# KaffinPX/neptune-core

Hardware: AMD Instinct MI355X
Metric: STARK proofs verified/sec (whole node) + Tip5 perms/sec vs VALU roofline (higher is better)
Workload: dtype u64 (Goldilocks mod p; XFE = cubic extension)

## Files before the change

### include/neptune_hip.h

```cpp
#ifndef NEPTUNE_HIP_H
#define NEPTUNE_HIP_H

#include <stddef.h>
#include <stdint.h>

#ifdef __cplusplus
extern "C" {
#endif

typedef struct nhip_ctx nhip_ctx;

enum {
    NHIP_OK = 0,
    NHIP_ERR_NO_DEVICE = 1,
    NHIP_ERR_HIP = 2,
    NHIP_ERR_OOM = 3,
    NHIP_ERR_ARG = 4,
    NHIP_ERR_DECODE = 5
};

#define NHIP_HW_QUEUES_RECOMMENDED 8
int nhip_init(uint32_t device_mask, nhip_ctx **out);
void nhip_destroy(nhip_ctx *ctx);
const char *nhip_strerror(int code);
// ... 53 lines not shown
} nhip_proof;

typedef struct {
    uint64_t num_proofs, proof_words;
    uint64_t tip5_perms_static;
    uint64_t tip5_perms_merkle;
    double ms_decode, ms_upload;
    double ms_fiat_shamir, ms_row_hash, ms_merkle, ms_ood_air, ms_fri, ms_deep, ms_device_total;
    double ms_merkle_hash;
    uint64_t merkle_hash_launches;
    double ms_mp_hash_kernel;
    uint64_t mp_hash_kernel_launches, mp_hash_kernel_perms;
    double ms_device_decode;
    double ms_mp_hash_exec;
    double ms_row_hash_exec;
} nhip_stats;

typedef struct nhip_air nhip_air;
typedef struct nhip_batch nhip_batch;

void nhip_stark_params_default(nhip_stark_params *out);
int nhip_air_create(const uint64_t *words, size_t n_words, nhip_air **out);
typedef struct {
    uint32_t lds_slots;
    uint32_t step_width;
    uint32_t slot_budget;
} nhip_air_options;
int nhip_air_create_ex(const uint64_t *words, size_t n_words, const nhip_air_options *options, nhip_air **out);
void nhip_air_destroy(nhip_air *air);
int nhip_air_info(const nhip_air *air, uint32_t *num_nodes, uint32_t *num_levels, uint32_t *num_constraints);
int nhip_air_slots(const nhip_air *air, uint32_t *lds_slots, uint32_t *global_slots);
int nhip_air_program(const nhip_air *air, uint32_t *step_off, size_t step_cap, uint32_t *ins, size_t ins_cap,
                     size_t *n_steps, size_t *n_ins);
int nhip_proof_decodes(const nhip_air *air, const nhip_stark_params *params, const nhip_claim *claim,
                       const nhip_proof *proof);
int nhip_host_alloc(size_t bytes, void **out);
int nhip_host_free(void *p);
int nhip_host_register(void *p, size_t bytes);
int nhip_host_unregister(void *p);
int nhip_host_alloc_near(nhip_ctx *ctx, size_t bytes, void **out);
int nhip_device_numa(nhip_ctx *ctx, int *numa_node, int *cpus, size_t cpu_cap, size_t *n_cpus);
int nhip_numa_from_sysfs(const char *sysfs_root, const char *pci_bus_id, int *numa_node, int *cpus, size_t cpu_cap,
                         size_t *n_cpus);
int nhip_cpulist_parse(const char *list, int *cpus, size_t cpu_cap, size_t *n_cpus);
int nhip_host_page_node(const void *ptr);
int nhip_set_host_threads(nhip_ctx *ctx, unsigned threads);
int nhip_verify_batch(nhip_ctx *ctx, nhip_air *air, const nhip_stark_params *params, const nhip_claim *claims,
                      const nhip_proof *proofs, size_t n, uint8_t *verdicts, nhip_stats *stats);
int nhip_batch_prepare(nhip_ctx *ctx, nhip_air *air, const nhip_stark_params *params, const nhip_claim *claims,
                       const nhip_proof *proofs, size_t n, nhip_batch **out);
int nhip_batch_refill(nhip_ctx *ctx, nhip_batch *batch, nhip_air *air, const nhip_stark_params *params,
                      const nhip_claim *claims, const nhip_proof *proofs, size_t n);
int nhip_batch_run(nhip_ctx *ctx, nhip_batch *batch, uint8_t *verdicts, uint8_t *all_ok);
int nhip_batch_launch(nhip_ctx *ctx, nhip_batch *batch);
int nhip_batch_wait(nhip_ctx *ctx, nhip_batch *batch, uint8_t *verdicts, uint8_t *all_ok);
int nhip_batch_stats(const nhip_batch *batch, nhip_stats *stats);
int nhip_batch_set_launch_timing(nhip_batch *batch, int on);
int nhip_batch_set_streams(nhip_batch *batch, int streams);
int nhip_batch_set_graph(nhip_batch *batch, int on);
int nhip_set_fs_form(int form);
int nhip_set_climb_from_ops(int64_t ops);
int nhip_batch_transcript(nhip_ctx *ctx, const nhip_batch *batch, size_t proof, uint64_t *xfe_out, size_t xfe_cap,
                          uint32_t *idx_out, size_t idx_cap, uint32_t *fail_bits, size_t *n_xfe);
void nhip_batch_destroy(nhip_batch *batch);

typedef struct nhip_queue nhip_queue;
// ... 221 lines not shown
```

### neptune-core_amd/csrc/stark_host.cpp

```cpp
#include <hip/hip_runtime.h>

#include <algorithm>
#include <atomic>
#include <chrono>
#include <cstdlib>
#include <cstring>
#include <memory>
#include <mutex>
#include <new>
#include <system_error>
#include <thread>
#include <vector>

#include "../../include/neptune_hip.h"
#include "device_scope.hpp"
#include "host_copy.hpp"
#include "host_numa.hpp"
#include "../../include/nhip_challenge_id.h"
#include "goldilocks.hpp"
#include "kernels.hpp"
#include "stark.hpp"
#include "wire.hpp"

using namespace nhip;
// ... 37 lines not shown
    static const bool on = [] {
        const char* v = nhip::ab_env("NHIP_STAGE_NT");
        return !v || std::strtol(v, nullptr, 10) != 0;
    }();
    return on;
}
unsigned host_threads(uint64_t bytes) {
    unsigned t = nhip::host_threads_env() ? nhip::host_threads_env() : std::thread::hardware_concurrency();
    t = std::max(1u, std::min(t, 16u));
    return bytes < (8ull << 20) ? 1u : t;
}

struct PinnedRanges {
    std::mutex mu;
    std::vector<std::pair<uintptr_t, size_t>> r;
    bool contains(const void* p, size_t bytes) {
        const uintptr_t a = (uintptr_t)p;
        std::lock_guard<std::mutex> g(mu);
        for (const auto& x : r)
            if (a >= x.first && a + bytes <= x.first + x.second && a + bytes >= a) return true;
        return false;
    }
};
PinnedRanges& pinned() {
    static PinnedRanges p;
    return p;
}

}

struct OodProgram {
    std::vector<OodIns> prog;
    std::vector<uint32_t> prog_off;
    std::vector<Xfe> consts;
    uint32_t slots = 0;
    uint32_t width = 0;
};

struct nhip_air {
    StarkDims dims_air{};
    std::vector<AirNode> nodes;
    std::vector<uint32_t> level_off;
    uint4 cons_off{};
    OodProgram progs[2];
    uint32_t lds_cap = AIR_LDS_SLOTS_MAX;
    struct Dev {
        int device;
        OodIns* d_prog[2];
        uint32_t* d_prog_off[2];
        Xfe* d_consts[2];
    };
    std::mutex mu;
    std::vector<Dev> devs;
};

struct VerifyScratch {
    std::mutex mu;
    void* dmem = nullptr;
    size_t dmem_bytes = 0;
    void* dwords = nullptr;
    size_t dwords_bytes = 0;
    void* draw = nullptr;
    size_t draw_bytes = 0;
    hipStream_t main = nullptr, aux = nullptr;
    hipEvent_t ev[STARK_EVENTS] = {};
    bool streams = false;
// ... 76 lines not shown
    d.num_checks = sp->num_collinearity_checks;
    d.num_deep = 3;
    d.log2_expansion = sp->log2_fri_expansion;
    d.num_trace_randomizers = sp->num_collinearity_checks + 2 * 3;
    d.num_sampled = air->dims_air.num_sampled;
    d.num_constraints = air->dims_air.num_constraints;
    D.expansion = 1u << sp->log2_fri_expansion;
    D.mont_words = sp->input_form == NHIP_INPUT_MONTGOMERY ? 1u : 0u;
    if (deep_rows8_lds_bytes(d) > 160 * 1024 - 8192) return false;
    if ((1ull << (log2_u64(d.num_checks) + 1 + d.log2_expansion)) > 4096) return false;
    return true;
}

int air_upload(nhip_ctx* ctx, nhip_air* a, nhip_air::Dev* out) {
    std::lock_guard<std::mutex> g(a->mu);
    const int device = nhip_internal_device(ctx);
    for (const auto& d : a->devs)
        if (d.device == device) {
            *out = d;
            return NHIP_OK;
        }
    nhip_air::Dev d{device, {nullptr, nullptr}, {nullptr, nullptr}, {nullptr, nullptr}};
    auto free_dev = [&]() {
        for (int k = 0; k < 2; ++k) {
            if (d.d_prog[k]) (void)hipFree(d.d_prog[k]);
            if (d.d_prog_off[k]) (void)hipFree(d.d_prog_off[k]);
            if (d.d_consts[k]) (void)hipFree(d.d_consts[k]);
        }
    };
    hipError_t e = hipSuccess;
    for (int k = 0; k < 2 && e == hipSuccess; ++k) {
        const OodProgram& pg = a->progs[k];
        e = hipMalloc(&d.d_prog[k], pg.prog.size() * sizeof(OodIns) + 16);
        if (e == hipSuccess) e = hipMalloc(&d.d_prog_off[k], pg.prog_off.size() * 4 + 4);
        if (e == hipSuccess) e = hipMalloc(&d.d_consts[k], pg.consts.size() * sizeof(Xfe) + 24);
        if (e == hipSuccess && !pg.prog.empty())
            e = hipMemcpy(d.d_prog[k], pg.prog.data(), pg.prog.size() * sizeof(OodIns), hipMemcpyHostToDevice);
        if (e == hipSuccess)
            e = hipMemcpy(d.d_prog_off[k], pg.prog_off.data(), pg.prog_off.size() * 4, hipMemcpyHostToDevice);
        if (e == hipSuccess && !pg.consts.empty())
            e = hipMemcpy(d.d_consts[k], pg.consts.data(), pg.consts.size() * sizeof(Xfe), hipMemcpyHostToDevice);
    }
    if (e != hipSuccess) {
        free_dev();
        return hipfail(e);
    }
    try {
        a->devs.reserve(a->devs.size() + 1);
    } catch (const std::bad_alloc&) {
        free_dev();
        return NHIP_ERR_OOM;
    }
    a->devs.push_back(d);
    *out = d;
    return NHIP_OK;
}

static constexpr uint32_t OOD_STEP_WIDTH = 512;

int ood_program_for(uint32_t n) {
    static const uint32_t lim = [] {
        const char* e = nhip::ab_env("NHIP_OOD_WIDE_PROG_MAX");
        return e ? (uint32_t)std::strtoul(e, nullptr, 10) : 1024u;
    }();
    return n <= lim ? 1 : 0;
}

void air_compile(const nhip_air* a, const std::vector<uint32_t>& cons, uint32_t width, uint32_t slot_budget,
                 OodProgram& pg) {
    pg = OodProgram{};
    pg.width = width;
    const size_t NN = a->nodes.size();
    const auto is_op = [&](size_t i) {
        const uint32_t op = a->nodes[i].op;
        return op == AIR_ADD || op == AIR_SUB || op == AIR_MUL;
    };
    std::vector<uint32_t> corder(NN, UINT32_MAX);
    {
        std::vector<uint32_t> st;
        for (size_t c = 0; c < cons.size(); ++c) {
            st.push_back(cons[c]);
            while (!st.empty()) {
                const uint32_t i = st.back();
                st.pop_back();
                if (corder[i] != UINT32_MAX) continue;
                corder[i] = (uint32_t)c;
                if (is_op(i)) {
                    st.push_back(a->nodes[i].a);
                    st.push_back(a->nodes[i].b);
                }
            }
// ... 35 lines not shown
    std::vector<uint32_t> free_slots, to_free;
    uint32_t next_slot = 0, live = 0;
    std::vector<OodIns> cur, acc_next;
    std::vector<std::pair<int32_t, uint64_t>> key(NN);
    auto retires = [&](uint32_t i) {
        if (!is_op(i)) return 0;
        const uint32_t x = a->nodes[i].a, y = a->nodes[i].b;
        int r = 0;
        if (slotted[x] && remaining[x] == (x == y ? 2u : 1u)) ++r;
        if (slotted[y] && y != x && remaining[y] == 1u) ++r;
        return r;
    };
    auto use = [&](uint32_t o) {
        if (slotted[o] && --remaining[o] == 0) to_free.push_back(ref[o]);
    };
    pg.prog_off.assign(1, 0);
    while (!ready.empty() || !acc_next.empty()) {
        cur.swap(acc_next);
        acc_next.clear();
        for (const OodIns& ins : cur)
            if (slotted[cons[ins.b]]) use(cons[ins.b]);
        for (uint32_t i : ready) key[i] = {-retires(i), ((uint64_t)corder[i] << 32) | i};
        std::sort(ready.begin(), ready.end(), [&](uint32_t x, uint32_t y) { return key[x] < key[y]; });
        const size_t room = width > cur.size() ? width - cur.size() : 1;
        std::vector<uint32_t> chosen, rest;
        for (uint32_t i : ready) {
            if (chosen.size() < room && (live < budget || key[i].first < 0 || chosen.empty())) {
                chosen.push_back(i);
                ++live;
            } else {
                rest.push_back(i);
            }
        }
        ready.swap(rest);
        for (uint32_t i : chosen) {
            uint32_t sl;
            if (!free_slots.empty()) {
                sl = free_slots.back();
                free_slots.pop_back();
            } else {
                sl = next_slot++;
            }
            const AirNode& nd = a->nodes[i];
            if (nd.op == AIR_INPUT) {
                cur.push_back(OodIns{OOD_LOAD, OOD_REF_INPUT | (nd.a << 27) | nd.b, 0, sl});
            } else if (nd.op == AIR_CONST) {
                cur.push_back(OodIns{OOD_LOAD, OOD_REF_CONST | cidx[i], 0, sl});
            } else {
                cur.push_back(OodIns{nd.op, ref[nd.a], ref[nd.b], sl});
                use(nd.a);
                use(nd.b);
            }
            ref[i] = OOD_REF_SLOT | sl;
            for (uint32_t c : acc_of[i]) acc_next.push_back(OodIns{OOD_ACC, ref[i], c, 0});
        }
        for (uint32_t i : chosen)
            for (uint32_t k = uoff[i]; k < uoff[i + 1]; ++k)
                if (--deps[users[k]] == 0) ready.push_back(users[k]);
        live -= (uint32_t)to_free.size();
        free_slots.insert(free_slots.end(), to_free.begin(), to_free.end());
        to_free.clear();
        auto kind_rank = [](uint32_t op) {
            return op == OOD_LOAD || op == OOD_ACC ? 0 : (op == AIR_MUL ? 1 : (op == AIR_ADD ? 2 : 3));
        };
        std::stable_sort(cur.begin(), cur.end(),
                         [&](const OodIns& x, const OodIns& y) { return kind_rank(x.op) < kind_rank(y.op); });
        pg.prog.insert(pg.prog.end(), cur.begin(), cur.end());
        pg.prog_off.push_back((uint32_t)pg.prog.size());
        cur.clear();
    }
    for (OodIns& ins : pg.prog)
        if (ins.op == OOD_ACC) ins.dst = next_slot + ins.b;
    pg.slots = next_slot + (uint32_t)cons.size();
}

inline size_t al(size_t x) { return (x + 255) & ~(size_t)255; }

inline size_t grown(size_t need, size_t have, bool refilled) {
    if (!refilled) return need;
    return std::max(need + need / 4, have ? 2 * have : 0);
}

}

extern "C" {

void nhip_stark_params_default(nhip_stark_params* out) {
    if (!out) return;
    out->security_level = 160;
    out->log2_fri_expansion = 2;
    out->num_collinearity_checks = 80;
    out->num_main = 379;
    out->num_aux = 88;
    out->num_quotient_segments = 4;
    out->input_form = NHIP_INPUT_CANONICAL;
}

int nhip_air_create(const uint64_t* w, size_t n, nhip_air** out) { return nhip_air_create_ex(w, n, nullptr, out); }

int nhip_air_create_ex(const uint64_t* w, size_t n, const nhip_air_options* opt, nhip_air** out) {
    if (!w || !out || n < 9) return NHIP_ERR_ARG;
    *out = nullptr;
    const nhip_air_options o = opt ? *opt : nhip_air_options{0, 0, 0};
// ... 84 lines not shown
    if (num_nodes) *num_nodes = (uint32_t)a->nodes.size();
    if (num_levels) *num_levels = (uint32_t)a->level_off.size() - 1;
    if (num_constraints) *num_constraints = a->dims_air.num_constraints;
    return NHIP_OK;
}

int nhip_air_slots(const nhip_air* a, uint32_t* lds_slots, uint32_t* global_slots) {
    if (!a) return NHIP_ERR_ARG;
    const uint32_t l = std::min<uint32_t>(a->progs[0].slots, a->lds_cap);
    if (lds_slots) *lds_slots = l;
    if (global_slots) *global_slots = a->progs[0].slots - l;
    return NHIP_OK;
}

int nhip_air_program(const nhip_air* a, uint32_t* step_off, size_t step_cap, uint32_t* ins, size_t ins_cap,
                     size_t* n_steps, size_t* n_ins) {
    if (!a) return NHIP_ERR_ARG;
    const OodProgram& pg = a->progs[0];
    const size_t ns = pg.prog_off.size() - 1, ni = pg.prog.size();
    if (n_steps) *n_steps = ns;
    if (n_ins) *n_ins = ni;
    if (step_off) {
        if (step_cap < ns + 1) return NHIP_ERR_ARG;
        std::memcpy(step_off, pg.prog_off.data(), (ns + 1) * 4);
    }
    if (ins) {
        if (ins_cap < 4 * ni) return NHIP_ERR_ARG;
        for (size_t i = 0; i < ni; ++i) {
            ins[4 * i] = pg.prog[i].op;
            ins[4 * i + 1] = pg.prog[i].a;
            ins[4 * i + 2] = pg.prog[i].b;
            ins[4 * i + 3] = pg.prog[i].dst;
        }
    }
    return NHIP_OK;
}

int nhip_proof_decodes(const nhip_air* air, const nhip_stark_params* sp, const nhip_claim* claim,
                       const nhip_proof* proof) {
    Dims D{};
    if (!claim || !proof || (proof->len && !proof->words) || !dims_from(sp, air, D)) return -NHIP_ERR_ARG;
    ProofDesc pd;
    FsOp ops[fs_ops_for(MAX_FRI_ROUNDS)];
    uint64_t perms, perms_lcw;
    const ClaimLoc cl{0, (uint32_t)claim->input_len, (uint32_t)claim->output_len};
    const uint32_t f = D.mont_words ? decode_stream<true>(proof->words, 0, proof->len, cl, D, pd, ops, perms, perms_lcw)
                                    : decode_stream<false>(proof->words, 0, proof->len, cl, D, pd, ops, perms, perms_lcw);
    return f ? 0 : 1;
}

namespace {
int batch_prepare(nhip_ctx* ctx, nhip_air* air, const nhip_stark_params* sp, const nhip_claim* claims,
                  const nhip_proof* proofs, const WireSrc* wire, size_t n, nhip_batch** out, VerifyScratch* scr,
                  nhip_batch* reuse = nullptr) {
    if (wire) {
        if (proofs || !sp || sp->input_form != NHIP_INPUT_CANONICAL) return NHIP_ERR_ARG;
        if ((wire->n_bytes && !wire->bytes) || (n && !wire->spans)) return NHIP_ERR_ARG;
        if (!wire_spans_ok(wire->spans, n, wire->n_bytes)) return NHIP_ERR_ARG;
    }
    if (!ctx || !out || (n && (!claims || (!proofs && !wire)))) return NHIP_ERR_ARG;
    if (reuse && (reuse->in_flight || reuse->scratch)) return NHIP_ERR_ARG;
    if (!reuse) *out = nullptr;
    Dims D{};
    if (!dims_from(sp, air, D)) return NHIP_ERR_ARG;
    if (n > 0xFFFFFFFFull) return NHIP_ERR_ARG;
    auto proof_len = [&](size_t i) -> uint64_t { return wire ? wire->spans[i].len : (uint64_t)proofs[i].len; };
// ... 903 lines not shown
```

### neptune-core_amd/csrc/stark_kernels.hip

```cpp
#include <hip/hip_ext.h>

#include <atomic>
#include <cstdlib>

#include "../../include/nhip_challenge_id.h"
#include "kernels.hpp"
#include "proof_codec.hpp"
#include "stark.hpp"
#include "tip5_device.hpp"
#include "xfe.hpp"

namespace nhip {

#ifndef NHIP_LAT_PRIO
#define NHIP_LAT_PRIO 2
#endif
__device__ __forceinline__ void latency_priority() {
    if constexpr (NHIP_LAT_PRIO > 0) __builtin_amdgcn_s_setprio(NHIP_LAT_PRIO);
}
static constexpr uint32_t AGE_PRIO_OLDEST = 2;
static constexpr uint32_t AGE_PRIO_MIN_PROOFS = 2048;
__device__ uint32_t g_batches_done;
struct AgePrio {
    uint32_t seq, k;
// ... 984 lines not shown
    return {(uint64_t)__shfl_xor((long long)v.c0, m), (uint64_t)__shfl_xor((long long)v.c1, m),
            (uint64_t)__shfl_xor((long long)v.c2, m)};
}

__device__ Xfe block_sum_xfe_waves(Xfe v, Xfe* sh) {
    const uint32_t tid = threadIdx.x, nw = blockDim.x >> 6;
#pragma unroll
    for (int m = 32; m > 0; m >>= 1) v = x_add(v, shfl_xor_xfe_fwd(v, m));
    if ((tid & 63u) == 0) sh[tid >> 6] = v;
    __syncthreads();
    Xfe r = sh[0];
    for (uint32_t w = 1; w < nw; ++w) r = x_add(r, sh[w]);
    __syncthreads();
    return r;
}

static constexpr uint32_t CH_COMPRESS_PROGRAM_DIGEST = NHIP_CH_CompressProgramDigestIndeterminate,
                          CH_STANDARD_INPUT = NHIP_CH_StandardInputIndeterminate,
                          CH_STANDARD_OUTPUT = NHIP_CH_StandardOutputIndeterminate,
                          CH_LOOKUP_TABLE_PUBLIC = NHIP_CH_LookupTablePublicIndeterminate;
static_assert(CH_LOOKUP_TABLE_PUBLIC == 54 && NHIP_CHALLENGE_SAMPLE_COUNT == 59 && NHIP_CHALLENGE_COUNT == 63,
              "triton-air ChallengeId layout");
static_assert(NHIP_CH_StandardInputTerminal == NHIP_CHALLENGE_SAMPLE_COUNT && NHIP_CH_CompressedProgramDigest == 62,
              "derived challenges follow the sampled ones");

__device__ __forceinline__ Xfe shfl_xor_xfe(Xfe v, int m) {
    return {(uint64_t)__shfl_xor((long long)v.c0, m), (uint64_t)__shfl_xor((long long)v.c1, m),
            (uint64_t)__shfl_xor((long long)v.c2, m)};
}

template <class Sym>
__device__ Xfe eval_terminal_wave(uint32_t n, Xfe c, Sym sym) {
    const uint32_t lane = threadIdx.x & 63u;
    const uint32_t ch = (n + 63u) / 64u;
    const uint32_t lo = min(n, lane * ch), hi = min(n, lo + ch);
    Xfe h = x_zero();
    for (uint32_t i = lo; i < hi; ++i) h = x_add(x_mul(h, c), x_lift(sym(i)));
    Xfe t = hi > lo ? x_mul(h, x_pow(c, n - hi)) : x_zero();
    if (lane == 0) t = x_add(t, x_pow(c, n));
#pragma unroll
    for (int m = 32; m > 0; m >>= 1) t = x_add(t, shfl_xor_xfe(t, m));
    return t;
}

#ifndef NHIP_OOD_WAVES
#define NHIP_OOD_WAVES 1
#endif

template <uint32_t BLOCK, bool MW, bool GS>
__global__ void __launch_bounds__(BLOCK, BLOCK == 256 ? NHIP_OOD_WAVES : 1) k_ood_air(const uint64_t* __restrict__ words, const ProofDesc* __restrict__ desc,
                                                 uint32_t n_proofs, StarkDims dims, const OodIns* __restrict__ prog,
                                                 const uint32_t* __restrict__ prog_off, uint32_t n_levels,
                                                 const Xfe* __restrict__ consts, uint4 cons_type_off,
                                                 const uint64_t* __restrict__ xs, uint64_t* __restrict__ ood_out,
                                                 uint32_t* __restrict__ fail, uint32_t lds_slots,
                                                 Xfe* __restrict__ gslots, uint32_t gslot_n) {
    latency_priority();
    extern __shared__ __attribute__((aligned(16))) unsigned char smem[];
    Xfe* red = reinterpret_cast<Xfe*>(smem);
    Xfe* zinv = red + 16;
    Xfe* chal_derived = zinv + 4;
    Xfe* misc = chal_derived + 4;
    uint32_t& zero_flag = *reinterpret_cast<uint32_t*>(misc + 4);
    Xfe* val = reinterpret_cast<Xfe*>(smem + AIR_LDS_HEADER);
    const uint32_t p = blockIdx.x, tid = threadIdx.x;
    Xfe* gval = gslots + (uint64_t)p * gslot_n;
    auto slot_ld = [&](uint32_t s) -> Xfe { return !GS || s < lds_slots ? val[s] : gval[s - lds_slots]; };
    auto slot_st = [&](uint32_t s, const Xfe& v) {
        if (!GS || s < lds_slots) val[s] = v;
        else gval[s - lds_slots] = v;
    };
    if (p >= n_proofs || (fail[p] & FAIL_DECODE)) return;
    const ProofDesc& d = desc[p];
    const SampleLayout sl = SampleLayout::of(dims, d.R);
    const uint64_t xb = d.xs_off * 3;
    const Xfe z = ld_xfe_raw(xs, xb + 3ull * sl.z);
    if (tid == 0) zero_flag = 0;
    __syncthreads();
    if (tid == 0) {
        const uint64_t w_inv = b_inv(root_of_unity(d.log2_ph));
        const Xfe except_last = x_sub(z, x_lift(w_inv));
        if (x_is_zero(except_last)) atomicOr(&zero_flag, 1u);
        misc[0] = except_last;
        zinv[3] = x_inv(except_last);
    } else if (tid == 64) {
        const Xfe zm1 = x_sub(z, x_one());
        if (x_is_zero(zm1)) atomicOr(&zero_flag, 1u);
        zinv[0] = x_inv(zm1);
    } else if (tid == 128) {
        Xfe zph = z;
        for (uint32_t q = 0; q < d.log2_ph; ++q) zph = x_mul(zph, zph);
        const Xfe cons = x_sub(zph, x_one());
        if (x_is_zero(cons)) atomicOr(&zero_flag, 1u);
        zinv[1] = x_inv(cons);
    } else if (tid >= 192 && tid < 256) {
        auto chal = [&](uint32_t i) { return ld_xfe_raw(xs, xb + 3ull * (sl.chal + i)); };
        const Xfe ein = eval_terminal_wave(d.claim_in_n, chal(CH_STANDARD_INPUT),
                                           [&](uint32_t i) { return word_mont<MW>(words[d.claim_in_off + i]); });
        const Xfe eout = eval_terminal_wave(d.claim_out_n, chal(CH_STANDARD_OUTPUT),
                                            [&](uint32_t i) { return word_mont<MW>(words[d.claim_out_off + i]); });
        const Xfe lut = eval_terminal_wave(256u, chal(CH_LOOKUP_TABLE_PUBLIC), [&](uint32_t i) {
            const uint64_t y = i + 1;
            return to_mont((y * y % 257u * y % 257u + 256u) % 257u);
        });
        const Xfe comp = eval_terminal_wave(5u, chal(CH_COMPRESS_PROGRAM_DIGEST),
                                            [&](uint32_t i) { return word_mont<MW>(words[d.claim_digest_off + i]); });
        if (tid == 192) {
            chal_derived[0] = ein;
            chal_derived[1] = eout;
            chal_derived[2] = lut;
            chal_derived[3] = comp;
        }
    }
    __syncthreads();
    if (tid == 0) zinv[2] = x_mul(misc[0], zinv[1]);
    __syncthreads();
    const uint32_t offs[5] = {0u, cons_type_off.x, cons_type_off.y, cons_type_off.z, cons_type_off.w};
    auto fetch = [&](uint32_t ref) -> Xfe {
        const uint32_t t = ref >> 30;
        if (t == 0) return slot_ld(ref);
        if (t == 1) return consts[ref & 0x3FFFFFFFu];
        const uint32_t kind = (ref >> 27) & 7u, i = ref & 0x7FFFFFFu;
        switch (kind) {
            case IN_MAIN_CURR: return ld_xfe_w<MW>(words, d.ood_mc + 3ull * i);
            case IN_AUX_CURR: return ld_xfe_w<MW>(words, d.ood_ac + 3ull * i);
            case IN_MAIN_NEXT: return ld_xfe_w<MW>(words, d.ood_mn + 3ull * i);
            case IN_AUX_NEXT: return ld_xfe_w<MW>(words, d.ood_an + 3ull * i);
            default:
                return i < dims.num_sampled ? ld_xfe_raw(xs, xb + 3ull * (sl.chal + i)) : chal_derived[i - dims.num_sampled];
        }
    };
    for (uint32_t lvl = 0; lvl < n_levels; ++lvl) {
        for (uint32_t q = prog_off[lvl] + tid; q < prog_off[lvl + 1]; q += blockDim.x) {
            const uint4 ins = reinterpret_cast<const uint4*>(prog)[q];
            if (ins.x >= OOD_LOAD) {
                slot_st(ins.w, fetch(ins.y));
            } else {
                const Xfe x = slot_ld(ins.y), y = slot_ld(ins.z);
                slot_st(ins.w, ins.x == OOD_ADD ? x_add(x, y) : (ins.x == OOD_SUB ? x_sub(x, y) : x_mul(x, y)));
            }
        }
        __syncthreads();
    }
    const uint32_t C = dims.num_constraints, cbase = lds_slots + gslot_n - C;
    Xfe acc = x_zero();
    for (uint32_t c = tid; c < C; c += blockDim.x) {
        uint32_t t = 0;
        while (t < 3 && c >= offs[t + 1]) ++t;
        const Xfe w = ld_xfe_raw(xs, xb + 3ull * (sl.quot_w + c));
        acc = x_add(acc, x_mul(w, x_mul(slot_ld(cbase + c), zinv[t])));
    }
    const Xfe ood_q = block_sum_xfe_waves(acc, red);
    const uint32_t M = dims.num_main, A = dims.num_aux, Q = dims.num_quot_seg;
    Xfe lc = x_zero(), ln = x_zero();
    for (uint32_t c = tid; c < M + A; c += blockDim.x) {
        const Xfe w = ld_xfe_raw(xs, xb + 3ull * (sl.lin_w + c));
        const Xfe vc = c < M ? ld_xfe_w<MW>(words, d.ood_mc + 3ull * c) : ld_xfe_w<MW>(words, d.ood_ac + 3ull * (c - M));
        const Xfe vn = c < M ? ld_xfe_w<MW>(words, d.ood_mn + 3ull * c) : ld_xfe_w<MW>(words, d.ood_an + 3ull * (c - M));
        lc = x_add(lc, x_mul(w, vc));
        ln = x_add(ln, x_mul(w, vn));
    }
    const Xfe sum_c = block_sum_xfe_waves(lc, red);
    const Xfe sum_n = block_sum_xfe_waves(ln, red);
    if (tid == 0) {
        Xfe seg = x_zero(), zk = x_one(), qlin = x_zero();
        for (uint32_t q = 0; q < Q; ++q) {
            const Xfe sq = ld_xfe_w<MW>(words, d.ood_qs + 3ull * q);
            seg = x_add(seg, x_mul(zk, sq));
            zk = x_mul(zk, z);
            qlin = x_add(qlin, x_mul(ld_xfe_raw(xs, xb + 3ull * (sl.lin_w + M + A + q)), sq));
        }
        uint32_t f = 0;
        if (zero_flag) f |= FAIL_ZERO_INVERSE;
        if (!x_eq(seg, ood_q)) f |= FAIL_OOD;
        if (f) atomicOr(&fail[p], f);
        uint64_t* o = ood_out + (uint64_t)p * 9;
        st_xfe_raw(o, 0, sum_c);
        st_xfe_raw(o, 3, sum_n);
        st_xfe_raw(o, 6, qlin);
    }
}

__device__ __forceinline__ uint64_t lds_pow(const uint64_t* __restrict__ sq, uint64_t e) {
    uint64_t r = MONT_ONE;
    for (uint32_t b = 0; e; ++b, e >>= 1)
        if (e & 1) r = mont_mul(r, sq[b]);
    return r;
}

#ifndef NHIP_FRI_WAVES
#define NHIP_FRI_WAVES 1
#endif
template <bool MW>
__device__ __forceinline__ void fri_body(uint32_t p, const uint64_t* __restrict__ words, const ProofDesc* __restrict__ desc,
                                         uint32_t n_proofs, StarkDims dims, const uint64_t* __restrict__ xs,
                                         const uint32_t* __restrict__ idx_all, uint64_t* __restrict__ xdom,
                                         uint32_t* __restrict__ fail) {
    __shared__ Xfe red[256];
    __shared__ uint64_t gsq[33], wsq[33];
    __shared__ uint32_t lflag;
    const uint32_t tid = threadIdx.x;
    if (p >= n_proofs || (fail[p] & FAIL_DECODE)) return;
    const ProofDesc& d = desc[p];
    const SampleLayout sl = SampleLayout::of(dims, d.R);
// ... 646 lines not shown
```

### neptune-core_amd/neptune_hip/_lib.py

```python
from __future__ import annotations

import ctypes
import os
import threading

import numpy as np

_HERE = os.path.dirname(os.path.abspath(__file__))
LIB_PATH = os.environ.get("NHIP_LIB") or os.path.join(_HERE, "libneptune_hip.so")

NHIP_OK = 0
NHIP_OK, NHIP_ERR_NO_DEVICE, NHIP_ERR_HIP, NHIP_ERR_OOM, NHIP_ERR_ARG, NHIP_ERR_DECODE = range(6)
_ERRORS = {1: "no HIP device", 2: "HIP runtime error", 3: "out of device memory", 4: "invalid argument",
           5: "malformed encoding"}

_u64p = np.ctypeslib.ndpointer(dtype=np.uint64, flags="C_CONTIGUOUS")
_u8p = np.ctypeslib.ndpointer(dtype=np.uint8, flags="C_CONTIGUOUS")
_vp = ctypes.c_void_p
_sz = ctypes.c_size_t

class StarkParams(ctypes.Structure):
    _fields_ = [("security_level", ctypes.c_uint32), ("log2_fri_expansion", ctypes.c_uint32),
                ("num_collinearity_checks", ctypes.c_uint32), ("num_main", ctypes.c_uint32),
                ("num_aux", ctypes.c_uint32), ("num_quotient_segments", ctypes.c_uint32),
# ... 91 lines not shown

_pp = ctypes.POINTER(ctypes.c_void_p)

SIGNATURES = {
    "nhip_init": ([ctypes.c_uint32, ctypes.POINTER(_vp)], ctypes.c_int),
    "nhip_destroy": ([_vp], None),
    "nhip_strerror": ([ctypes.c_int], ctypes.c_char_p),
    "nhip_device_ordinal": ([_vp], ctypes.c_int),
    "nhip_abi_version": ([], ctypes.c_int),
    "nhip_tip5_permutation": ([_vp, _u64p, _sz], ctypes.c_int),
    "nhip_tip5_hash_pair": ([_vp, _u64p, _u64p, _sz, _u64p], ctypes.c_int),
    "nhip_tip5_hash_varlen": ([_vp, _u64p, _u64p, _sz, _u64p], ctypes.c_int),
    "nhip_mtree_build": ([_vp, _u64p, _sz, _u64p], ctypes.c_int),
    "nhip_mtree_verify": ([_vp, _u64p, _sz, _u64p, _u64p, _u64p, ctypes.c_uint32, _sz, _u8p], ctypes.c_int),
    "nhip_dev_alloc": ([_vp, _sz, ctypes.POINTER(_vp)], ctypes.c_int),
    "nhip_dev_free": ([_vp, _vp], ctypes.c_int),
    "nhip_memcpy_h2d": ([_vp, _vp, _vp, _sz], ctypes.c_int),
    "nhip_memcpy_d2h": ([_vp, _vp, _vp, _sz], ctypes.c_int),
    "nhip_synchronize": ([_vp], ctypes.c_int),
    "nhip_tip5_permutation_dev": ([_vp, _vp, _sz], ctypes.c_int),
    "nhip_tip5_hash_pair_dev": ([_vp, _vp, _vp, _sz, _vp], ctypes.c_int),
    "nhip_tip5_hash_varlen_dev": ([_vp, _vp, _vp, _sz, _vp], ctypes.c_int),
    "nhip_mtree_build_dev": ([_vp, _vp, _sz, _vp], ctypes.c_int),
    "nhip_mtree_verify_dev": ([_vp, _vp, _sz, _vp, _vp, _vp, ctypes.c_uint32, _sz, _vp], ctypes.c_int),
    "nhip_verdicts_all_dev": ([_vp, _vp, _sz, ctypes.POINTER(ctypes.c_uint8)], ctypes.c_int),
    "nhip_stark_params_default": ([ctypes.POINTER(StarkParams)], None),
    "nhip_air_create": ([_u64p, _sz, _pp], ctypes.c_int),
    "nhip_air_create_ex": ([_u64p, _sz, ctypes.c_void_p, _pp], ctypes.c_int),
    "nhip_air_destroy": ([_vp], None),
    "nhip_air_info": ([_vp, ctypes.POINTER(ctypes.c_uint32), ctypes.POINTER(ctypes.c_uint32),
                       ctypes.POINTER(ctypes.c_uint32)], ctypes.c_int),
    "nhip_air_program": ([_vp, ctypes.c_void_p, _sz, ctypes.c_void_p, _sz, ctypes.POINTER(_sz), ctypes.POINTER(_sz)],
                         ctypes.c_int),
    "nhip_air_slots": ([_vp, ctypes.POINTER(ctypes.c_uint32), ctypes.POINTER(ctypes.c_uint32)], ctypes.c_int),
    "nhip_proof_from_be_bytes": ([ctypes.c_void_p, _sz, ctypes.c_void_p, _sz, ctypes.POINTER(_sz)], ctypes.c_int),
    "nhip_proof_to_be_bytes": ([ctypes.c_void_p, _sz, ctypes.c_void_p], ctypes.c_int),
    "nhip_claim_hash": ([_vp, ctypes.POINTER(Claim), _u64p], ctypes.c_int),
    "nhip_queue_create": ([_vp, _vp, ctypes.POINTER(StarkParams), ctypes.c_uint32, ctypes.c_uint32,
                           ctypes.POINTER(_vp)], ctypes.c_int),
    "nhip_queue_verify": ([_vp, _vp, _vp, _sz, _vp], ctypes.c_int),
    "nhip_queue_stats": ([_vp, ctypes.POINTER(ctypes.c_uint64), ctypes.POINTER(ctypes.c_uint64)], ctypes.c_int),
    "nhip_queue_profile_read": ([_vp, ctypes.POINTER(QueueProfile), ctypes.c_int], ctypes.c_int),
    "nhip_queue_destroy": ([_vp], None),
    "nhip_host_alloc": ([_sz, ctypes.POINTER(_vp)], ctypes.c_int),
    "nhip_host_free": ([_vp], ctypes.c_int),
    "nhip_host_register": ([_vp, _sz], ctypes.c_int),
    "nhip_host_alloc_near": ([_vp, _sz, ctypes.POINTER(_vp)], ctypes.c_int),
    "nhip_device_numa": ([_vp, ctypes.POINTER(ctypes.c_int), ctypes.POINTER(ctypes.c_int), _sz,
                          ctypes.POINTER(_sz)], ctypes.c_int),
    "nhip_numa_from_sysfs": ([ctypes.c_char_p, ctypes.c_char_p, ctypes.POINTER(ctypes.c_int),
                              ctypes.POINTER(ctypes.c_int), _sz, ctypes.POINTER(_sz)], ctypes.c_int),
    "nhip_cpulist_parse": ([ctypes.c_char_p, ctypes.POINTER(ctypes.c_int), _sz, ctypes.POINTER(_sz)], ctypes.c_int),
    "nhip_host_page_node": ([_vp], ctypes.c_int),
    "nhip_set_host_threads": ([_vp, ctypes.c_uint], ctypes.c_int),
    "nhip_host_unregister": ([_vp], ctypes.c_int),
    "nhip_pow_mast_commit": ([_vp, ctypes.c_void_p, ctypes.c_void_p], ctypes.c_int),
    "nhip_pow_preprocess": ([_vp, ctypes.c_uint32, ctypes.c_void_p, ctypes.c_int, ctypes.c_void_p,
                             ctypes.POINTER(_vp)], ctypes.c_int),
    "nhip_pow_buffer_destroy": ([_vp], None),
    "nhip_pow_buffer_root": ([_vp, _vp, ctypes.c_void_p], ctypes.c_int),
    "nhip_pow_buffer_leaf": ([_vp, _vp, ctypes.c_uint64, ctypes.c_void_p], ctypes.c_int),
    "nhip_pow_buffer_path": ([_vp, _vp, ctypes.c_uint64, ctypes.c_void_p], ctypes.c_int),
    "nhip_pow_guess_batch": ([_vp, _vp, ctypes.c_void_p, ctypes.c_void_p, ctypes.c_void_p, _sz, ctypes.c_void_p,
                              ctypes.c_void_p, ctypes.c_void_p, ctypes.c_void_p], ctypes.c_int),
    "nhip_pow_validate_batch": ([_vp, ctypes.c_uint32, ctypes.c_void_p, ctypes.c_void_p, ctypes.c_void_p,
                                 ctypes.c_void_p, ctypes.c_void_p, ctypes.c_void_p, ctypes.c_void_p, ctypes.c_void_p,
# ... 114 lines not shown
```

### neptune-core_amd/neptune_hip/stark.py

```python
from __future__ import annotations

import ctypes
import dataclasses
from dataclasses import dataclass, field
from typing import List, Sequence, Tuple

import numpy as np

from . import _lib
from ._lib import check


@dataclass
class Stark:
    security_level: int = 160
    log2_fri_expansion: int = 2
    num_collinearity_checks: int = 80
    num_main: int = 379
    num_aux: int = 88
    num_quotient_segments: int = 4
    input_form: int = _lib.NHIP_INPUT_CANONICAL

    def c(self) -> _lib.StarkParams:
        return _lib.StarkParams(self.security_level, self.log2_fri_expansion, self.num_collinearity_checks,
# ... 51 lines not shown
    version: int = 0
    input: Sequence[int] = field(default_factory=list)
    output: Sequence[int] = field(default_factory=list)


class Air:

    def __init__(self, words: Sequence[int], lds_slots: int = 0, step_width: int = 0, slot_budget: int = 0):
        self.lib = _lib.load()
        w = np.ascontiguousarray(np.asarray(words, dtype=np.uint64))
        h = ctypes.c_void_p()
        opts = (ctypes.c_uint32 * 3)(lds_slots, step_width, slot_budget)
        check(self.lib.nhip_air_create_ex(w, w.size, ctypes.cast(opts, ctypes.c_void_p), ctypes.byref(h)),
              "nhip_air_create_ex")
        self.handle = h.value

    def info(self):
        a, b, c = ctypes.c_uint32(), ctypes.c_uint32(), ctypes.c_uint32()
        check(self.lib.nhip_air_info(self.handle, ctypes.byref(a), ctypes.byref(b), ctypes.byref(c)), "air_info")
        lds, glob = ctypes.c_uint32(), ctypes.c_uint32()
        check(self.lib.nhip_air_slots(self.handle, ctypes.byref(lds), ctypes.byref(glob)), "air_slots")
        return {"nodes": a.value, "levels": b.value, "constraints": c.value, "lds_slots": lds.value,
                "global_slots": glob.value}

    def program(self):
        ns, ni = ctypes.c_size_t(), ctypes.c_size_t()
        check(self.lib.nhip_air_program(self.handle, None, 0, None, 0, ctypes.byref(ns), ctypes.byref(ni)),
              "nhip_air_program")
        off = np.zeros(ns.value + 1, dtype=np.uint32)
        ins = np.zeros((max(ni.value, 1), 4), dtype=np.uint32)
        check(self.lib.nhip_air_program(self.handle, off.ctypes.data, off.size, ins.ctypes.data, ins.size,
                                        ctypes.byref(ns), ctypes.byref(ni)), "nhip_air_program")
        return off, ins[:ni.value]

    def __del__(self):
        try:
            if self.handle:
                self.lib.nhip_air_destroy(self.handle)
        except Exception:
            pass


class _Marshal:

    def __init__(self, claims: Sequence[Claim], proofs: Sequence[Sequence[int]]):
        n = len(claims)
        self.keep = []
        self.claims = (_lib.Claim * max(n, 1))()
        self.proofs = (_lib.Proof * max(n, 1))()
        u64 = ctypes.POINTER(ctypes.c_uint64)
        for i, (c, pw) in enumerate(zip(claims, proofs)):
            inp = np.ascontiguousarray(np.asarray(list(c.input), dtype=np.uint64))
            out = np.ascontiguousarray(np.asarray(list(c.output), dtype=np.uint64))
            pa = np.ascontiguousarray(np.asarray(pw, dtype=np.uint64))
            self.keep += [inp, out, pa]
            cc = self.claims[i]
            for k in range(5):
                cc.program_digest[k] = int(c.program_digest[k])
            cc.version = int(c.version)
            cc.input = inp.ctypes.data_as(u64) if inp.size else None
            cc.input_len = inp.size
            cc.output = out.ctypes.data_as(u64) if out.size else None
            cc.output_len = out.size
            self.proofs[i].words = pa.ctypes.data_as(u64) if pa.size else None
            self.proofs[i].len = pa.size
        self.n = n
# ... 562 lines not shown
```

### neptune-core_amd/rust/neptune-hip-sys/src/lib.rs

```rust
#![allow(non_camel_case_types)]
#![no_std]

use core::ffi::{c_char, c_int, c_uint, c_void};

pub const NHIP_OK: c_int = 0;
pub const NHIP_ERR_NO_DEVICE: c_int = 1;
pub const NHIP_ERR_HIP: c_int = 2;
pub const NHIP_ERR_OOM: c_int = 3;
pub const NHIP_ERR_ARG: c_int = 4;
pub const NHIP_ERR_DECODE: c_int = 5;

pub const NHIP_BLOCK_PROOF_GENESIS: u32 = 0;
pub const NHIP_BLOCK_PROOF_INVALID: u32 = 1;
pub const NHIP_BLOCK_PROOF_SINGLE: u32 = 2;
pub const NHIP_TX_PROOF_COLLECTION: u32 = 0;
pub const NHIP_TX_SINGLE_PROOF: u32 = 1;
pub const NHIP_INPUT_CANONICAL: u32 = 0;
pub const NHIP_INPUT_MONTGOMERY: u32 = 1;
pub const NHIP_HW_QUEUES_RECOMMENDED: u32 = 8;

macro_rules! opaque {
    ($($name:ident),*) => { $( #[repr(C)] pub struct $name { _p: [u8; 0] } )* };
}
opaque!(nhip_ctx, nhip_air, nhip_batch, nhip_group, nhip_group_stream, nhip_queue, nhip_pow_buffer, nhip_arena);
// ... 204 lines not shown
    pub fn nhip_abi_version() -> c_int;
    pub fn nhip_tip5_permutation(ctx: *mut nhip_ctx, states: *mut u64, n: usize) -> c_int;
    pub fn nhip_tip5_hash_pair(ctx: *mut nhip_ctx, left: *const u64, right: *const u64, n: usize,
                               out: *mut u64) -> c_int;
    pub fn nhip_tip5_hash_varlen(ctx: *mut nhip_ctx, data: *const u64, offsets: *const u64, n: usize,
                                 out: *mut u64) -> c_int;
    pub fn nhip_mtree_build(ctx: *mut nhip_ctx, leafs: *const u64, n_leafs: usize, nodes_out: *mut u64) -> c_int;
    pub fn nhip_mtree_verify(ctx: *mut nhip_ctx, roots: *const u64, n_roots: usize, indices: *const u64,
                             leafs: *const u64, paths: *const u64, depth: u32, n: usize, verdicts: *mut u8) -> c_int;
    pub fn nhip_dev_alloc(ctx: *mut nhip_ctx, bytes: usize, dptr: *mut *mut c_void) -> c_int;
    pub fn nhip_dev_free(ctx: *mut nhip_ctx, dptr: *mut c_void) -> c_int;
    pub fn nhip_memcpy_h2d(ctx: *mut nhip_ctx, dst: *mut c_void, src: *const c_void, bytes: usize) -> c_int;
    pub fn nhip_memcpy_d2h(ctx: *mut nhip_ctx, dst: *mut c_void, src: *const c_void, bytes: usize) -> c_int;
    pub fn nhip_synchronize(ctx: *mut nhip_ctx) -> c_int;
    pub fn nhip_tip5_permutation_dev(ctx: *mut nhip_ctx, d_states: *mut u64, n: usize) -> c_int;
    pub fn nhip_tip5_hash_pair_dev(ctx: *mut nhip_ctx, d_left: *const u64, d_right: *const u64, n: usize,
                                   d_out: *mut u64) -> c_int;
    pub fn nhip_tip5_hash_varlen_dev(ctx: *mut nhip_ctx, d_data: *const u64, d_offsets: *const u64, n: usize,
                                     d_out: *mut u64) -> c_int;
    pub fn nhip_mtree_build_dev(ctx: *mut nhip_ctx, d_leafs: *const u64, n_leafs: usize, d_nodes: *mut u64) -> c_int;
    pub fn nhip_mtree_verify_dev(ctx: *mut nhip_ctx, d_roots: *const u64, n_roots: usize,
                                 d_indices: *const u64, d_leafs: *const u64, d_paths: *const u64, depth: u32,
                                 n: usize, d_verdicts: *mut u8) -> c_int;
    pub fn nhip_verdicts_all_dev(ctx: *mut nhip_ctx, d_verdicts: *const u8, n: usize, all_ok: *mut u8) -> c_int;
    pub fn nhip_stark_params_default(out: *mut nhip_stark_params);
    pub fn nhip_air_create(words: *const u64, n_words: usize, out: *mut *mut nhip_air) -> c_int;
    pub fn nhip_air_create_ex(words: *const u64, n_words: usize, options: *const nhip_air_options,
                              out: *mut *mut nhip_air) -> c_int;
    pub fn nhip_air_destroy(air: *mut nhip_air);
    pub fn nhip_air_info(air: *const nhip_air, num_nodes: *mut u32, num_levels: *mut u32,
                         num_constraints: *mut u32) -> c_int;
    pub fn nhip_air_program(air: *const nhip_air, step_off: *mut u32, step_cap: usize, ins: *mut u32, ins_cap: usize,
                            n_steps: *mut usize, n_ins: *mut usize) -> c_int;
    pub fn nhip_air_slots(air: *const nhip_air, lds_slots: *mut u32, global_slots: *mut u32) -> c_int;
    pub fn nhip_proof_decodes(air: *const nhip_air, params: *const nhip_stark_params,
                              claim: *const nhip_claim, proof: *const nhip_proof) -> c_int;
    pub fn nhip_host_alloc(bytes: usize, out: *mut *mut c_void) -> c_int;
    pub fn nhip_host_free(p: *mut c_void) -> c_int;
    pub fn nhip_host_register(p: *mut c_void, bytes: usize) -> c_int;
    pub fn nhip_host_alloc_near(ctx: *mut nhip_ctx, bytes: usize, out: *mut *mut c_void) -> c_int;
    pub fn nhip_device_numa(ctx: *mut nhip_ctx, numa_node: *mut c_int, cpus: *mut c_int, cpu_cap: usize,
                            n_cpus: *mut usize) -> c_int;
    pub fn nhip_numa_from_sysfs(sysfs_root: *const c_char, pci_bus_id: *const c_char, numa_node: *mut c_int,
                                cpus: *mut c_int, cpu_cap: usize, n_cpus: *mut usize) -> c_int;
    pub fn nhip_cpulist_parse(list: *const c_char, cpus: *mut c_int, cpu_cap: usize, n_cpus: *mut usize) -> c_int;
    pub fn nhip_host_page_node(ptr: *const c_void) -> c_int;
    pub fn nhip_set_host_threads(ctx: *mut nhip_ctx, threads: c_uint) -> c_int;
    pub fn nhip_host_unregister(p: *mut c_void) -> c_int;
    pub fn nhip_verify_batch(ctx: *mut nhip_ctx, air: *mut nhip_air, params: *const nhip_stark_params,
                             claims: *const nhip_claim, proofs: *const nhip_proof, n: usize,
                             verdicts: *mut u8, stats: *mut nhip_stats) -> c_int;
    pub fn nhip_batch_prepare(ctx: *mut nhip_ctx, air: *mut nhip_air, params: *const nhip_stark_params,
                              claims: *const nhip_claim, proofs: *const nhip_proof, n: usize,
                              out: *mut *mut nhip_batch) -> c_int;
    pub fn nhip_batch_refill(ctx: *mut nhip_ctx, batch: *mut nhip_batch, air: *mut nhip_air,
                             params: *const nhip_stark_params, claims: *const nhip_claim,
                             proofs: *const nhip_proof, n: usize) -> c_int;
    pub fn nhip_batch_run(ctx: *mut nhip_ctx, batch: *mut nhip_batch, verdicts: *mut u8, all_ok: *mut u8) -> c_int;
    pub fn nhip_batch_launch(ctx: *mut nhip_ctx, batch: *mut nhip_batch) -> c_int;
    pub fn nhip_batch_wait(ctx: *mut nhip_ctx, batch: *mut nhip_batch, verdicts: *mut u8, all_ok: *mut u8) -> c_int;
    pub fn nhip_batch_stats(batch: *const nhip_batch, stats: *mut nhip_stats) -> c_int;
    pub fn nhip_batch_transcript(ctx: *mut nhip_ctx, batch: *const nhip_batch, proof: usize,
                                 xfe_out: *mut u64, xfe_cap: usize, idx_out: *mut u32, idx_cap: usize,
                                 fail_bits: *mut u32, n_xfe: *mut usize) -> c_int;
    pub fn nhip_batch_destroy(batch: *mut nhip_batch);
    pub fn nhip_set_fs_form(form: c_int) -> c_int;
// ... 121 lines not shown
```

Measured before the change: 458,400.

## Segment OOD AIR program by op kind and parallelize OOD prologue/epilogue

The OOD AIR compiler now splits each step into load, multiply and add/sub segments, and the scheduler rounds multiplies per step to a quota of 64 so the mul segment fills whole waves. The kernel then runs branch-free loops per segment instead of dispatching on op per instruction. Separately, the three zerofier inverses are merged into one batched inversion on a single thread, terminal evaluations are spread across three waves with a log-depth Horner combine, and the final quotient-segment sum runs across 64 lanes with a shuffle reduction instead of a serial loop. These changes target warp divergence and serial single-thread work, at the cost of a more complex scheduler and possibly more steps.

```diff
diff --git a/include/neptune_hip.h b/include/neptune_hip.h
--- a/include/neptune_hip.h
+++ b/include/neptune_hip.h
@@ -109,6 +109,7 @@
 int nhip_air_slots(const nhip_air *air, uint32_t *lds_slots, uint32_t *global_slots);
 int nhip_air_program(const nhip_air *air, uint32_t *step_off, size_t step_cap, uint32_t *ins, size_t ins_cap,
                      size_t *n_steps, size_t *n_ins);
+int nhip_air_segments(const nhip_air *air, uint32_t *seg_off, size_t seg_cap, size_t *n_bounds);
 int nhip_proof_decodes(const nhip_air *air, const nhip_stark_params *params, const nhip_claim *claim,
                        const nhip_proof *proof);
 int nhip_host_alloc(size_t bytes, void **out);
diff --git a/neptune-core_amd/csrc/stark_host.cpp b/neptune-core_amd/csrc/stark_host.cpp
--- a/neptune-core_amd/csrc/stark_host.cpp
+++ b/neptune-core_amd/csrc/stark_host.cpp
@@ -93,6 +93,7 @@
 struct OodProgram {
     std::vector<OodIns> prog;
     std::vector<uint32_t> prog_off;
+    std::vector<uint32_t> seg_off;
     std::vector<Xfe> consts;
     uint32_t slots = 0;
     uint32_t width = 0;
@@ -235,12 +236,12 @@
     for (int k = 0; k < 2 && e == hipSuccess; ++k) {
         const OodProgram& pg = a->progs[k];
         e = hipMalloc(&d.d_prog[k], pg.prog.size() * sizeof(OodIns) + 16);
-        if (e == hipSuccess) e = hipMalloc(&d.d_prog_off[k], pg.prog_off.size() * 4 + 4);
+        if (e == hipSuccess) e = hipMalloc(&d.d_prog_off[k], pg.seg_off.size() * 4 + 4);
         if (e == hipSuccess) e = hipMalloc(&d.d_consts[k], pg.consts.size() * sizeof(Xfe) + 24);
         if (e == hipSuccess && !pg.prog.empty())
             e = hipMemcpy(d.d_prog[k], pg.prog.data(), pg.prog.size() * sizeof(OodIns), hipMemcpyHostToDevice);
         if (e == hipSuccess)
-            e = hipMemcpy(d.d_prog_off[k], pg.prog_off.data(), pg.prog_off.size() * 4, hipMemcpyHostToDevice);
+            e = hipMemcpy(d.d_prog_off[k], pg.seg_off.data(), pg.seg_off.size() * 4, hipMemcpyHostToDevice);
         if (e == hipSuccess && !pg.consts.empty())
             e = hipMemcpy(d.d_consts[k], pg.consts.data(), pg.consts.size() * sizeof(Xfe), hipMemcpyHostToDevice);
     }
@@ -260,6 +261,7 @@
 }
 
 static constexpr uint32_t OOD_STEP_WIDTH = 512;
+static constexpr uint32_t OOD_MUL_QUOTA = 64;
 
 int ood_program_for(uint32_t n) {
     static const uint32_t lim = [] {
@@ -361,6 +363,38 @@
                 rest.push_back(i);
             }
         }
+        {
+            const auto is_mul = [&](uint32_t i) { return a->nodes[i].op == AIR_MUL; };
+            size_t muls = 0;
+            for (uint32_t i : chosen) muls += is_mul(i);
+            size_t drop = muls % OOD_MUL_QUOTA;
+            if (drop && (muls > drop || chosen.size() > muls)) {
+                std::vector<uint32_t> kept, back;
+                for (size_t k = chosen.size(); k-- > 0;) {
+                    const uint32_t i = chosen[k];
+                    if (drop && is_mul(i) && key[i].first == 0) {
+                        back.push_back(i);
+                        --drop;
+                        --live;
+                    } else {
+                        kept.push_back(i);
+                    }
+                }
+                std::reverse(kept.begin(), kept.end());
+                chosen.swap(kept);
+                std::vector<uint32_t> rest2;
+                for (uint32_t i : rest) {
+                    if (!is_mul(i) && chosen.size() < room && (live < budget || key[i].first < 0)) {
+                        chosen.push_back(i);
+                        ++live;
+                    } else {
+                        rest2.push_back(i);
+                    }
+                }
+                rest.swap(rest2);
+                rest.insert(rest.end(), back.begin(), back.end());
+            }
+        }
         ready.swap(rest);
         for (uint32_t i : chosen) {
             uint32_t sl;
@@ -394,10 +428,16 @@
         };
         std::stable_sort(cur.begin(), cur.end(),
                          [&](const OodIns& x, const OodIns& y) { return kind_rank(x.op) < kind_rank(y.op); });
+        uint32_t bound = (uint32_t)pg.prog.size();
+        for (int rank = 0; rank < 3; ++rank) {
+            pg.seg_off.push_back(bound);
+            for (const OodIns& ins : cur) bound += kind_rank(ins.op) == rank || (rank == 2 && kind_rank(ins.op) == 3);
+        }
         pg.prog.insert(pg.prog.end(), cur.begin(), cur.end());
         pg.prog_off.push_back((uint32_t)pg.prog.size());
         cur.clear();
     }
+    pg.seg_off.push_back((uint32_t)pg.prog.size());
     for (OodIns& ins : pg.prog)
         if (ins.op == OOD_ACC) ins.dst = next_slot + ins.b;
     pg.slots = next_slot + (uint32_t)cons.size();
@@ -548,6 +588,17 @@
             ins[4 * i + 2] = pg.prog[i].b;
             ins[4 * i + 3] = pg.prog[i].dst;
         }
+    }
+    return NHIP_OK;
+}
+
+int nhip_air_segments(const nhip_air* a, uint32_t* seg_off, size_t seg_cap, size_t* n_bounds) {
+    if (!a) return NHIP_ERR_ARG;
+    const OodProgram& pg = a->progs[0];
+    if (n_bounds) *n_bounds = pg.seg_off.size();
+    if (seg_off) {
+        if (seg_cap < pg.seg_off.size()) return NHIP_ERR_ARG;
+        std::memcpy(seg_off, pg.seg_off.data(), pg.seg_off.size() * 4);
     }
     return NHIP_OK;
 }
diff --git a/neptune-core_amd/csrc/stark_kernels.hip b/neptune-core_amd/csrc/stark_kernels.hip
--- a/neptune-core_amd/csrc/stark_kernels.hip
+++ b/neptune-core_amd/csrc/stark_kernels.hip
@@ -1040,15 +1040,26 @@
 template <class Sym>
 __device__ Xfe eval_terminal_wave(uint32_t n, Xfe c, Sym sym) {
     const uint32_t lane = threadIdx.x & 63u;
-    const uint32_t ch = (n + 63u) / 64u;
-    const uint32_t lo = min(n, lane * ch), hi = min(n, lo + ch);
-    Xfe h = x_zero();
-    for (uint32_t i = lo; i < hi; ++i) h = x_add(x_mul(h, c), x_lift(sym(i)));
-    Xfe t = hi > lo ? x_mul(h, x_pow(c, n - hi)) : x_zero();
-    if (lane == 0) t = x_add(t, x_pow(c, n));
-#pragma unroll
-    for (int m = 32; m > 0; m >>= 1) t = x_add(t, shfl_xor_xfe(t, m));
-    return t;
+    uint32_t s = 0;
+    while (s < 6u && (1u << s) < n + 1u) ++s;
+    const uint32_t L = 1u << s, ch = (n + L) >> s, pad = L * ch - n;
+    auto entry = [&](uint32_t pos) -> Xfe {
+        if (lane >= L) return x_zero();
+        if (pos >= pad) return x_lift(sym(pos - pad));
+        return pos + 1u == pad ? x_one() : x_zero();
+    };
+    Xfe h = entry(lane * ch), m = c;
+    for (uint32_t k = 1; k < ch; ++k) {
+        h = x_add(x_mul(h, c), entry(lane * ch + k));
+        m = x_mul(m, c);
+    }
+    for (uint32_t k = 0; k < s; ++k) {
+        const Xfe o = shfl_xor_xfe(h, 1 << k);
+        const bool up = (lane >> k) & 1u;
+        h = x_add(x_mul(up ? o : h, m), up ? h : o);
+        if (k + 1u < s) m = x_mul(m, m);
+    }
+    return h;
 }
 
 #ifndef NHIP_OOD_WAVES
@@ -1058,7 +1069,7 @@
 template <uint32_t BLOCK, bool MW, bool GS>
 __global__ void __launch_bounds__(BLOCK, BLOCK == 256 ? NHIP_OOD_WAVES : 1) k_ood_air(const uint64_t* __restrict__ words, const ProofDesc* __restrict__ desc,
                                                  uint32_t n_proofs, StarkDims dims, const OodIns* __restrict__ prog,
-                                                 const uint32_t* __restrict__ prog_off, uint32_t n_levels,
+                                                 const uint32_t* __restrict__ seg_off, uint32_t n_levels,
                                                  const Xfe* __restrict__ consts, uint4 cons_type_off,
                                                  const uint64_t* __restrict__ xs, uint64_t* __restrict__ ood_out,
                                                  uint32_t* __restrict__ fail, uint32_t lds_slots,
@@ -1088,40 +1099,45 @@
     if (tid == 0) {
         const uint64_t w_inv = b_inv(root_of_unity(d.log2_ph));
         const Xfe except_last = x_sub(z, x_lift(w_inv));
-        if (x_is_zero(except_last)) atomicOr(&zero_flag, 1u);
-        misc[0] = except_last;
-        zinv[3] = x_inv(except_last);
-    } else if (tid == 64) {
         const Xfe zm1 = x_sub(z, x_one());
-        if (x_is_zero(zm1)) atomicOr(&zero_flag, 1u);
-        zinv[0] = x_inv(zm1);
-    } else if (tid == 128) {
         Xfe zph = z;
         for (uint32_t q = 0; q < d.log2_ph; ++q) zph = x_mul(zph, zph);
         const Xfe cons = x_sub(zph, x_one());
-        if (x_is_zero(cons)) atomicOr(&zero_flag, 1u);
-        zinv[1] = x_inv(cons);
-    } else if (tid >= 192 && tid < 256) {
+        const bool z0 = x_is_zero(zm1), z1 = x_is_zero(cons), z3 = x_is_zero(except_last);
+        if (z0 || z1 || z3) zero_flag = 1u;
+        const Xfe a = z0 ? x_one() : zm1, b = z1 ? x_one() : cons, c = z3 ? x_one() : except_last;
+        const Xfe ab = x_mul(a, b);
+        const Xfe iabc = x_inv(x_mul(ab, c));
+        const Xfe iab = x_mul(iabc, c);
+        const Xfe i1 = z1 ? x_zero() : x_mul(iab, a);
+        zinv[0] = z0 ? x_zero() : x_mul(iab, b);
+        zinv[1] = i1;
+        zinv[2] = x_mul(except_last, i1);
+        zinv[3] = z3 ? x_zero() : x_mul(iabc, ab);
+    } else if (tid >= 64 && tid < 256) {
         auto chal = [&](uint32_t i) { return ld_xfe_raw(xs, xb + 3ull * (sl.chal + i)); };
-        const Xfe ein = eval_terminal_wave(d.claim_in_n, chal(CH_STANDARD_INPUT),
-                                           [&](uint32_t i) { return word_mont<MW>(words[d.claim_in_off + i]); });
-        const Xfe eout = eval_terminal_wave(d.claim_out_n, chal(CH_STANDARD_OUTPUT),
-                                            [&](uint32_t i) { return word_mont<MW>(words[d.claim_out_off + i]); });
-        const Xfe lut = eval_terminal_wave(256u, chal(CH_LOOKUP_TABLE_PUBLIC), [&](uint32_t i) {
-            const uint64_t y = i + 1;
-            return to_mont((y * y % 257u * y % 257u + 256u) % 257u);
-        });
-        const Xfe comp = eval_terminal_wave(5u, chal(CH_COMPRESS_PROGRAM_DIGEST),
-                                            [&](uint32_t i) { return word_mont<MW>(words[d.claim_digest_off + i]); });
-        if (tid == 192) {
-            chal_derived[0] = ein;
-            chal_derived[1] = eout;
-            chal_derived[2] = lut;
-            chal_derived[3] = comp;
-        }
-    }
-    __syncthreads();
-    if (tid == 0) zinv[2] = x_mul(misc[0], zinv[1]);
+        const uint32_t wv = tid >> 6;
+        if (wv == 1) {
+            const Xfe lut = eval_terminal_wave(256u, chal(CH_LOOKUP_TABLE_PUBLIC), [&](uint32_t i) {
+                const uint64_t y = i + 1;
+                return to_mont((y * y % 257u * y % 257u + 256u) % 257u);
+            });
+            if (tid == 64) chal_derived[2] = lut;
+        } else if (wv == 2) {
+            const Xfe ein = eval_terminal_wave(d.claim_in_n, chal(CH_STANDARD_INPUT),
+                                               [&](uint32_t i) { return word_mont<MW>(words[d.claim_in_off + i]); });
+            const Xfe comp = eval_terminal_wave(5u, chal(CH_COMPRESS_PROGRAM_DIGEST),
+                                                [&](uint32_t i) { return word_mont<MW>(words[d.claim_digest_off + i]); });
+            if (tid == 128) {
+                chal_derived[0] = ein;
+                chal_derived[3] = comp;
+            }
+        } else {
+            const Xfe eout = eval_terminal_wave(d.claim_out_n, chal(CH_STANDARD_OUTPUT),
+                                                [&](uint32_t i) { return word_mont<MW>(words[d.claim_out_off + i]); });
+            if (tid == 192) chal_derived[1] = eout;
+        }
+    }
     __syncthreads();
     const uint32_t offs[5] = {0u, cons_type_off.x, cons_type_off.y, cons_type_off.z, cons_type_off.w};
     auto fetch = [&](uint32_t ref) -> Xfe {
@@ -1139,14 +1155,20 @@
         }
     };
     for (uint32_t lvl = 0; lvl < n_levels; ++lvl) {
-        for (uint32_t q = prog_off[lvl] + tid; q < prog_off[lvl + 1]; q += blockDim.x) {
+        const uint32_t s0 = seg_off[3 * lvl], s1 = seg_off[3 * lvl + 1], s2 = seg_off[3 * lvl + 2],
+                       s3 = seg_off[3 * lvl + 3];
+        for (uint32_t q = s0 + tid; q < s1; q += blockDim.x) {
             const uint4 ins = reinterpret_cast<const uint4*>(prog)[q];
-            if (ins.x >= OOD_LOAD) {
-                slot_st(ins.w, fetch(ins.y));
-            } else {
-                const Xfe x = slot_ld(ins.y), y = slot_ld(ins.z);
-                slot_st(ins.w, ins.x == OOD_ADD ? x_add(x, y) : (ins.x == OOD_SUB ? x_sub(x, y) : x_mul(x, y)));
-            }
+            slot_st(ins.w, fetch(ins.y));
+        }
+        for (uint32_t q = s1 + tid; q < s2; q += blockDim.x) {
+            const uint4 ins = reinterpret_cast<const uint4*>(prog)[q];
+            slot_st(ins.w, x_mul(slot_ld(ins.y), slot_ld(ins.z)));
+        }
+        for (uint32_t q = s2 + tid; q < s3; q += blockDim.x) {
+            const uint4 ins = reinterpret_cast<const uint4*>(prog)[q];
+            const Xfe x = slot_ld(ins.y), y = slot_ld(ins.z);
+            slot_st(ins.w, ins.x == OOD_ADD ? x_add(x, y) : x_sub(x, y));
         }
         __syncthreads();
     }
@@ -1170,14 +1192,27 @@
     }
     const Xfe sum_c = block_sum_xfe_waves(lc, red);
     const Xfe sum_n = block_sum_xfe_waves(ln, red);
-    if (tid == 0) {
-        Xfe seg = x_zero(), zk = x_one(), qlin = x_zero();
-        for (uint32_t q = 0; q < Q; ++q) {
+    if (tid >= 64) return;
+    Xfe seg = x_zero(), qlin = x_zero();
+    for (uint32_t base = 0; base < Q; base += 64u) {
+        const uint32_t q = base + tid, top = min(Q - 1u, base + 63u);
+        Xfe zk = (q & 1u) ? z : x_one(), zp = z;
+        for (uint32_t e = top >> 1, bit = 1; e; e >>= 1, ++bit) {
+            zp = x_mul(zp, zp);
+            zk = x_mul(zk, ((q >> bit) & 1u) ? zp : x_one());
+        }
+        if (q < Q) {
             const Xfe sq = ld_xfe_w<MW>(words, d.ood_qs + 3ull * q);
             seg = x_add(seg, x_mul(zk, sq));
-            zk = x_mul(zk, z);
             qlin = x_add(qlin, x_mul(ld_xfe_raw(xs, xb + 3ull * (sl.lin_w + M + A + q)), sq));
         }
+    }
+#pragma unroll
+    for (int m = 32; m > 0; m >>= 1) {
+        seg = x_add(seg, shfl_xor_xfe(seg, m));
+        qlin = x_add(qlin, shfl_xor_xfe(qlin, m));
+    }
+    if (tid == 0) {
         uint32_t f = 0;
         if (zero_flag) f |= FAIL_ZERO_INVERSE;
         if (!x_eq(seg, ood_q)) f |= FAIL_OOD;
diff --git a/neptune-core_amd/neptune_hip/_lib.py b/neptune-core_amd/neptune_hip/_lib.py
--- a/neptune-core_amd/neptune_hip/_lib.py
+++ b/neptune-core_amd/neptune_hip/_lib.py
@@ -147,6 +147,7 @@
                        ctypes.POINTER(ctypes.c_uint32)], ctypes.c_int),
     "nhip_air_program": ([_vp, ctypes.c_void_p, _sz, ctypes.c_void_p, _sz, ctypes.POINTER(_sz), ctypes.POINTER(_sz)],
                          ctypes.c_int),
+    "nhip_air_segments": ([_vp, ctypes.c_void_p, _sz, ctypes.POINTER(_sz)], ctypes.c_int),
     "nhip_air_slots": ([_vp, ctypes.POINTER(ctypes.c_uint32), ctypes.POINTER(ctypes.c_uint32)], ctypes.c_int),
     "nhip_proof_from_be_bytes": ([ctypes.c_void_p, _sz, ctypes.c_void_p, _sz, ctypes.POINTER(_sz)], ctypes.c_int),
     "nhip_proof_to_be_bytes": ([ctypes.c_void_p, _sz, ctypes.c_void_p], ctypes.c_int),
diff --git a/neptune-core_amd/neptune_hip/stark.py b/neptune-core_amd/neptune_hip/stark.py
--- a/neptune-core_amd/neptune_hip/stark.py
+++ b/neptune-core_amd/neptune_hip/stark.py
@@ -107,6 +107,14 @@
         check(self.lib.nhip_air_program(self.handle, off.ctypes.data, off.size, ins.ctypes.data, ins.size,
                                         ctypes.byref(ns), ctypes.byref(ni)), "nhip_air_program")
         return off, ins[:ni.value]
+
+    def segments(self):
+        n = ctypes.c_size_t()
+        check(self.lib.nhip_air_segments(self.handle, None, 0, ctypes.byref(n)), "nhip_air_segments")
+        seg = np.zeros(n.value, dtype=np.uint32)
+        check(self.lib.nhip_air_segments(self.handle, seg.ctypes.data, seg.size, ctypes.byref(n)), "nhip_air_segments")
+        steps = (n.value - 1) // 3
+        return np.stack([seg[k:k + 3 * steps:3] for k in range(3)] + [seg[3::3]], axis=1)
 
     def __del__(self):
         try:
diff --git a/neptune-core_amd/rust/neptune-hip-sys/src/lib.rs b/neptune-core_amd/rust/neptune-hip-sys/src/lib.rs
--- a/neptune-core_amd/rust/neptune-hip-sys/src/lib.rs
+++ b/neptune-core_amd/rust/neptune-hip-sys/src/lib.rs
@@ -260,6 +260,7 @@
                          num_constraints: *mut u32) -> c_int;
     pub fn nhip_air_program(air: *const nhip_air, step_off: *mut u32, step_cap: usize, ins: *mut u32, ins_cap: usize,
                             n_steps: *mut usize, n_ins: *mut usize) -> c_int;
+    pub fn nhip_air_segments(air: *const nhip_air, seg_off: *mut u32, seg_cap: usize, n_bounds: *mut usize) -> c_int;
     pub fn nhip_air_slots(air: *const nhip_air, lds_slots: *mut u32, global_slots: *mut u32) -> c_int;
     pub fn nhip_proof_decodes(air: *const nhip_air, params: *const nhip_stark_params,
                               claim: *const nhip_claim, proof: *const nhip_proof) -> c_int;
```

Result: faster. 468,100 (median of 6 runs) (+2.1%).
